# StephenTaf/Modern-Search-Engines-Project

Measured on AMD Instinct MI355X. Metric: queries/sec, two-stage retrieval top-100 (BM25 top-1000 + dense full scan + rerank/fuse), higher is better.
Workload: dtype f32 (exact f32 cosines of every returned document; candidates filtered by one pass of f16 products with a measured margin; batches <= 64 queries: f16x2-split products, |err| <= 8e-6) (dense cosine) / f64 (BM25, fuse)

## Files before the change

modern-search-engines-project_amd/csrc/msr_dense_ks.hip:

```cpp
#include <stdlib.h>

#include "msr_common.h"
#include "msr_internal.h"
#include "msr_frag.h"

namespace {

template <int QB, int MODE, int RING_DOCS = MSR_WIDE_RING, int NWAVES = 8> struct KsCfg {
    static constexpr int WAVES = NWAVES;
    static constexpr int THREADS = WAVES * 64;
    static constexpr int KS = MSR_DIM / 32;
    static constexpr int KT = KS / WAVES;
    static constexpr int PIECES = MODE == MODE_BF16 ? 1 : 2;
    static constexpr int NLU = MODE == MODE_BF16 ? KT : 2 * KT;
    static constexpr int ROW16 = MODE == MODE_BF16 ? MSR_DIM * 2 / 16 : MSR_DIM * 4 / 16;
    static constexpr int NQ = 16 * QB;
    static constexpr int RING = RING_DOCS;
    static constexpr int SWZ = (NQ < 64 ? NQ : 64) - 1;
    static constexpr int TILE = QB * 64 * 4;
    static constexpr int PER = QB / 2;
    static constexpr size_t p_bytes = (size_t)2 * WAVES * TILE * 4;
    static constexpr size_t r_bytes = (size_t)RING * NQ * 4;
    static constexpr size_t total = p_bytes + r_bytes;
    static_assert(QB == 2 || QB == 4 || QB == 8, "the reduction hands QB / 2 floats (one tile column piece) to a lane");
// ... 240 lines not shown
    }
}

int scan_debug_flags() {
#ifdef MSR_DIAG
    static const int v = [] { const char* e = getenv("MSR_SCAN_DEBUG"); return e ? atoi(e) : 0; }();
    return v;
#else
    return 0;
#endif
}

int ks_pipe_knob(int dflt) {
#ifdef MSR_DIAG
    static const char* v = getenv("MSR_KS_PIPE");
    return v ? atoi(v) : dflt;
#else
    return dflt;
#endif
}

template <int QB, int MODE, int NBUF, int PIPE = 1, int RING_DOCS = MSR_WIDE_RING, int NWAVES = 8>
hipError_t launch_ksplit(const DenseIndex& ix, const void* emb, const float* qn, int nq, float* docscore,
                         hipStream_t stream, int n_slices = 1, void* qimg_slices = nullptr) {
    using L = KsCfg<QB, MODE, RING_DOCS, NWAVES>;
    static_assert(L::total <= 160 * 1024, "LDS budget");
    hipError_t err = hipFuncSetAttribute((const void*)dense_ksplit_kernel<QB, MODE, NBUF, PIPE, RING_DOCS, NWAVES>,
                                         hipFuncAttributeMaxDynamicSharedMemorySize, (int)L::total);
    if (err != hipSuccess) return err;
    void* qimg = qimg_slices ? qimg_slices : ix.qimg;
    err = msr_build_qimage(MODE == MODE_PRE ? MODE_F16X2 : MODE, qn, QB * n_slices, qimg, stream);
    if (err != hipSuccess) return err;
    dense_ksplit_kernel<QB, MODE, NBUF, PIPE, RING_DOCS, NWAVES><<<dim3((unsigned)ix.n_spans, (unsigned)n_slices), L::THREADS,
                                                                 L::total, stream>>>(
        ix, emb, (const f32x4*)qimg, nq, docscore, scan_debug_flags());
    return hipGetLastError();
}

}

hipError_t msr_pack_row_meta(const int32_t* chunk_doc, const float* inv_norm, int64_t n, void* row_meta,
                             hipStream_t stream) {
    if (n <= 0) return hipSuccess;
    pack_row_meta_kernel<<<(unsigned)((n + 16 + 255) / 256), 256, 0, stream>>>(chunk_doc, inv_norm, n, (int2*)row_meta);
    return hipGetLastError();
}

hipError_t msr_presplit_rows(const float* src, int64_t n_rows, void* dst, hipStream_t stream) {
    if (n_rows <= 0) return hipSuccess;
    presplit_kernel<<<16384, 256, 0, stream>>>(src, n_rows, (f32x4*)dst);
    return hipGetLastError();
}

hipError_t msr_dense_scan_ksplit(const DenseIndex& ix, DensePlan plan, const float* qn, int nq, float* docscore,
// ... 4 lines not shown
        case dense_case(DENSE_KSPLIT_F16X2, 2): return launch_ksplit<2, MODE_F16X2, 3, 0>(ix, rows, qn, nq, docscore, stream);
        case dense_case(DENSE_KSPLIT_F16X2, 4):
#ifdef MSR_DIAG
            if (ks_pipe_knob(0) == 2) return launch_ksplit<4, MODE_F16X2, 3, 2>(ix, rows, qn, nq, docscore, stream);
            if (ks_pipe_knob(0) == 8) return launch_ksplit<4, MODE_F16X2, 3, 0>(ix, rows, qn, nq, docscore, stream);
#endif
            return launch_ksplit<4, MODE_F16X2, 2, 0, MSR_WIDE_RING, 12>(ix, rows, qn, nq, docscore, stream);
        case dense_case(DENSE_KSPLIT_PRESPLIT, 2): return launch_ksplit<2, MODE_PRE, 3, 0>(ix, rows, qn, nq, docscore, stream);
        case dense_case(DENSE_KSPLIT_PRESPLIT, 4): return launch_ksplit<4, MODE_PRE, 2, 0, MSR_WIDE_RING, 12>(ix, rows, qn, nq, docscore, stream);
        case dense_case(DENSE_KSPLIT_EXACT, 2): return launch_ksplit<2, MODE_F32, 3, 0>(ix, rows, qn, nq, docscore, stream);
        case dense_case(DENSE_KSPLIT_EXACT, 4): return launch_ksplit<4, MODE_F32, 2, 0, MSR_WIDE_RING, 12>(ix, rows, qn, nq, docscore, stream);
        case dense_case(DENSE_BF16_KSPLIT, 4):
#ifdef MSR_DIAG
            if (!ks_pipe_knob(1)) return launch_ksplit<4, MODE_BF16, 4, 0>(ix, rows, qn, nq, docscore, stream);
#endif
            return launch_ksplit<4, MODE_BF16, 4, 1>(ix, rows, qn, nq, docscore, stream);
        case dense_case(DENSE_BF16_KSPLIT, 8): return launch_ksplit<8, MODE_BF16, 3, 0, 64>(ix, rows, qn, nq, docscore, stream);
        default: break;
    }
    return hipErrorInvalidValue;
}

size_t msr_ksplit_slice_image_bytes() { return (size_t)4 * KsCfg<4, MODE_F16X2, MSR_WIDE_RING, 12>::KS * 2 * 64 * 16; }
hipError_t msr_dense_scan_slices(const DenseIndex& ix, const float* qn, int nq, float* docscore, void* qimg_slices,
                                 hipStream_t stream) {
    if (nq <= 0 || ix.n_docs <= 0) return hipSuccess;
    if (!dense_stream_bound(dense_binding(ix), true) || !ix.row_meta || !ix.gate || !qimg_slices) return hipErrorInvalidValue;
    static_assert(MSR_DENSE_FALLBACK_SLICE == 16 * 4, "a slice is what the QB = 4 instance below takes");
    return launch_ksplit<4, MODE_F16X2, 2, 0, MSR_WIDE_RING, 12>(ix, ix.emb, qn, nq, docscore, stream, dense_fallback_slices(nq),
                                                                 qimg_slices);
}
```

modern-search-engines-project_amd/csrc/msr_engine.hip:

```cpp
#include <hip/hip_runtime.h>
#include <stdarg.h>
#include <stdio.h>
#include <stdlib.h>
#include <string.h>

#include <algorithm>
#include <new>
#include <vector>

#include "../../include/msretr.h"
#include "msr_devmem.h"
#include "msr_internal.h"
#include "msr_match_args.h"

struct HipMem {
    static hipError_t alloc(void** p, size_t bytes) { return hipMalloc(p, bytes); }
    static void free(void* p) { (void)hipFree(p); }
};
using Group = DevGroup<HipMem>;

struct msr_engine {
    msr_config cfg;
    char err[512];
    Group mem_engine;
// ... 1315 lines not shown
                              (hipStream_t)stream));
    return MSR_OK;
}

extern "C" int msr_union_candidates(msr_engine* e, int32_t n_queries, const int32_t* lex_doc, const double* lex_score,
                                    const int32_t* lex_n, int32_t k_lex, const int32_t* dense_doc, const double* dense_bm25,
                                    const int32_t* dense_n, int32_t k_dense, int32_t* out_doc, double* out_score, int32_t* out_src,
                                    int32_t* out_n, int32_t max_cand, void* stream) {
    if (!e) return MSR_ERR_INVALID;
    if (n_queries < 0 || k_lex < 0 || k_lex > MSR_MAX_K || k_dense < 0 || k_dense > MSR_MAX_K || max_cand < 1 ||
        (int64_t)k_lex + k_dense > max_cand)
        return fail(e, MSR_ERR_INVALID, "msr_union_candidates: bad argument (k_lex=%d, k_dense=%d: each in [0, %d], their sum <= "
                    "max_cand=%d)", k_lex, k_dense, MSR_MAX_K, max_cand);
    if (!out_doc || !out_score || !out_src || !out_n || (k_lex > 0 && (!lex_doc || !lex_score || !lex_n)) ||
        (k_dense > 0 && (!dense_doc || !dense_bm25 || !dense_n)))
        return fail(e, MSR_ERR_INVALID, "msr_union_candidates: bad argument (NULL list)");
    if (n_queries == 0) return MSR_OK;
    HIP_TRY(e, hipSetDevice(e->cfg.device));
    HIP_TRY(e, msr_union_lists(n_queries, lex_doc, lex_score, lex_n, k_lex, dense_doc, dense_bm25, dense_n, k_dense, out_doc,
                               out_score, out_src, out_n, max_cand, (hipStream_t)stream));
    return MSR_OK;
}

static int dense_gated_fallback(msr_engine* e, int nq, int k, int32_t* out_doc, float* out_score, int32_t* out_chunk,
                                int32_t* out_n, hipStream_t st) {
    const int64_t N = e->dense.n_docs;
    DenseIndex ix = e->dense;
    ix.gate = e->gf_gate;
    HIP_TRY(e, msr_dense_scan_slices(ix, e->gf_qn, nq, (float*)e->score_rows, e->gf_fb_qimg, st));
    SelScratch sel = e->sel;
    sel.gate = e->gf_gate; sel.gate_per64 = 1;
    HIP_TRY(e, msr_select_topk(32, e->score_rows, N, e->dense.score_stride, nq, k, sel, out_doc, out_score, out_n, st));
    ix.gate = e->gf_gate; ix.gate_per64 = 1;
    if (out_chunk) HIP_TRY(e, msr_best_chunk(ix, e->gf_qn, nq, k, 0, out_doc, out_n, out_chunk, st));
    return MSR_OK;
}

static hipEvent_t* pass_events(msr_engine* e, int kind, hipEvent_t ev[4]) {
    if (!e->timing || e->ev_count[kind] >= msr_engine::EV_RING || e->ev_count[3] >= msr_engine::EV_RING) return nullptr;
    ev[0] = e->ev_start[3][e->ev_count[3]]; ev[1] = e->ev_stop[3][e->ev_count[3]];
    ev[2] = e->ev_start[kind][e->ev_count[kind]]; ev[3] = e->ev_stop[kind][e->ev_count[kind]];
    return ev;
}
static void pass_events_used(msr_engine* e, int kind, const hipEvent_t* ev) {
    if (ev) { e->ev_count[kind]++; e->ev_count[3]++; }
}

extern "C" int msr_dense_split_max(const msr_engine* e, int32_t k) {
    if (!e || !e->have_chunks || k < 1 || k > e->cfg.max_k ||
        !dense_stream_ok(dense_binding(e->dense), 0, e->gf_ok, e->gf.n_tiles, k))
        return 0;
    return e->gf.caps.call_cap;
}

extern "C" int msr_dense_topk_begin(msr_engine* e, const float* q, int32_t n_queries, int32_t k, int32_t k_part, float* out_part,
                                    void* stream) {
    if (!e) return MSR_ERR_INVALID;
    if (!e->have_chunks) return fail(e, MSR_ERR_NOT_BOUND, "msr_dense_topk_begin: chunks not bound");
    if (e->split_pending) return fail(e, MSR_ERR_INVALID, "msr_dense_topk_begin: the previous begin has not been ended");
    const int cap = msr_dense_split_max(e, k);
    if (!q || !out_part || k_part < 1 || k_part > k || n_queries <= 64 || n_queries > cap)
        return fail(e, MSR_ERR_INVALID, "msr_dense_topk_begin: needs 64 < n_queries <= msr_dense_split_max() = %d, 1 <= k_part <= k (got %d, %d, %d)",
                    cap, n_queries, k_part, k);
    hipStream_t st = (hipStream_t)stream;
    HIP_TRY(e, hipSetDevice(e->cfg.device));
    HIP_TRY(e, msr_prep_queries(q, n_queries, e->gf_qn, dense_fallback_pad(n_queries), st));
    HIP_TRY(e, hipMemsetAsync(e->gf_gate, 0, GF_GATE_BYTES, st));
    hipEvent_t ev_buf[4];
    hipEvent_t* ev = pass_events(e, 0, ev_buf);
    int width = 0;
    int segs = 0;
    HIP_TRY(e, msr_gemm_f32_pass(e->gf, e->dense, e->gf_qn, n_queries, k, k_part, out_part, ev, &width, &segs, st));
    e->last_dense_width = width;
    e->last_dense_segments = segs;
    pass_events_used(e, 0, ev);
    e->split_pending = n_queries;
    return MSR_OK;
}

extern "C" int msr_dense_topk_end(msr_engine* e, int32_t n_queries, int32_t k, const float* bound, int32_t* out_doc,
                                  float* out_score, int32_t* out_chunk, int32_t* out_n, void* stream) {
    if (!e) return MSR_ERR_INVALID;
    if (!e->have_chunks) return fail(e, MSR_ERR_NOT_BOUND, "msr_dense_topk_end: chunks not bound");
    if (!e->gf_ok || e->split_pending != n_queries || n_queries <= 0)
        return fail(e, MSR_ERR_INVALID, "msr_dense_topk_end: no matching msr_dense_topk_begin (pending %d, got %d)", e->split_pending, n_queries);
    if (!out_doc || !out_score || !out_n || k < 1 || k > e->cfg.max_k) return fail(e, MSR_ERR_INVALID, "msr_dense_topk_end: bad argument");
    e->split_pending = 0;
    hipStream_t st = (hipStream_t)stream;
    HIP_TRY(e, hipSetDevice(e->cfg.device));
    HIP_TRY(e, msr_gemm_f32_finish(e->gf, e->dense, e->gf_qn, n_queries, k, bound, out_doc, out_score, out_chunk, out_n, e->gf_gate, st));
// ... 34 lines not shown
                                      out_n + s0, out_chunk + (int64_t)s0 * k, st));
    }
    return MSR_OK;
}

extern "C" int msr_dense_topk(msr_engine* e, const float* q, int32_t n_queries, int32_t k, int32_t max_chunks_per_doc,
                              int32_t* out_doc, float* out_score, int32_t* out_chunk, int32_t* out_n, void* stream) {
    if (!e) return MSR_ERR_INVALID;
    const bool args_ok = dense_topk_args(e, n_queries, k, max_chunks_per_doc, q, out_doc, out_score, out_n);
    if (const int rc = dense_entry_ok(e, "msr_dense_topk", false, args_ok, k)) return rc;
    if (n_queries == 0) return MSR_OK;
    hipStream_t st = (hipStream_t)stream;
    HIP_TRY(e, hipSetDevice(e->cfg.device));
    const DenseBinding b = dense_binding(e->dense);
    const int slice = dense_slice(b, max_chunks_per_doc);
    const bool gemm = dense_stream_ok(b, max_chunks_per_doc, e->gf_ok, e->gf.n_tiles, k);
    e->last_dense_width = gemm && n_queries > slice ? 0 : slice;
    e->last_dense_segments = 0;
    int q0 = 0;
    while (q0 < n_queries) {
        const int left = n_queries - q0;
        if (gemm && left > slice) {
            const int nq = std::min(e->gf.caps.call_cap, left);
            HIP_TRY(e, msr_prep_queries(q + (int64_t)q0 * MSR_DIM, nq, e->gf_qn, dense_fallback_pad(nq), st));
            HIP_TRY(e, hipMemsetAsync(e->gf_gate, 0, GF_GATE_BYTES, st));
            hipEvent_t ev_buf[4];
            hipEvent_t* ev = pass_events(e, 0, ev_buf);
            int width = 0, segs = 0;
            HIP_TRY(e, msr_gemm_f32_topk(e->gf, e->dense, e->gf_qn, nq, k, out_doc + (int64_t)q0 * k,
                                         out_score + (int64_t)q0 * k, out_chunk ? out_chunk + (int64_t)q0 * k : nullptr,
                                         out_n + q0, e->gf_gate, ev, &width, &segs, st));
            e->last_dense_width = std::max(e->last_dense_width, width);
            e->last_dense_segments = segs;
            pass_events_used(e, 0, ev);
            {
                int rcf = dense_gated_fallback(e, nq, k, out_doc + (int64_t)q0 * k, out_score + (int64_t)q0 * k,
                                               out_chunk ? out_chunk + (int64_t)q0 * k : nullptr, out_n + q0, st);
                if (rcf) return rcf;
            }
            q0 += nq;
        } else {
            const int nq = std::min(slice, left);
            int rc = dense_sweeps(e, q, q0, nq, k, max_chunks_per_doc, nullptr, out_doc, out_score, out_chunk, out_n, st, nullptr);
            if (rc) return rc;
            q0 += nq;
        }
    }
    return MSR_OK;
// ... 511 lines not shown
```

modern-search-engines-project_amd/csrc/msr_gemm_f32.hip:

```cpp
#include <cmath>
#include <type_traits>

#include "msr_common.h"
#include "msr_internal.h"
#include "msr_frag.h"
#include "msr_gemm_dev.h"

namespace {

constexpr int GF_THREADS = 512;
constexpr int GF_KT = MSR_DIM / 32;
constexpr int GF_ROWB = MSR_DIM * 4;
constexpr int GF_PAIR_CAP = 4096;

typedef StreamArgs GemmF32Args;

__device__ __forceinline__ const char* uniform_ptr(const char* p) {
    const uint64_t u = (uint64_t)p;
    const uint32_t lo = __builtin_amdgcn_readfirstlane((uint32_t)u), hi = __builtin_amdgcn_readfirstlane((uint32_t)(u >> 32));
    return (const char*)(((uint64_t)hi << 32) | lo);
}

constexpr int GS_NB = 8;
constexpr int GS_STEP = 8192;
// ... 637 lines not shown
    if (i >= GF_KT * 256 * 4) return;
    const int g = blockIdx.y;
    const int cp = i & 3, ql = (i >> 2) & 255, kt = i >> 10;
    const int q = 256 * g + ql;
    const int c = cp ^ (((ql >> 3) & 1) << 1);
    f16x8 h;
    if (q < nq) {
        const float* src = qn + (size_t)q * MSR_DIM + (BF16 ? 64 * (kt >> 1) + 16 * c + 8 * (kt & 1) : 32 * kt + 8 * c);
        if (TOBF16) {
            bf16x8 b;
#pragma unroll
            for (int j = 0; j < 8; ++j) b[j] = (__bf16)src[j];
            h = __builtin_bit_cast(f16x8, b);
        } else {
            h = cvt_f16_rtn(*(const f32x4*)src, *(const f32x4*)(src + 4));
        }
    } else {
#pragma unroll
        for (int j = 0; j < 8; ++j) h[j] = (_Float16)0.f;
    }
    qimg[(size_t)g * (GF_KT * 256 * 4) + i] = h;
}

__global__ __launch_bounds__(256) void build_qimg1_kernel(const float* __restrict__ qn, int nq, f16x8* __restrict__ qimg) {
    const int i = blockIdx.x * 256 + threadIdx.x;
    if (i >= GF_KT * 128 * 4) return;
    const int g = blockIdx.y;
    const int cp = i & 3, ql = (i >> 2) & 127, kt = i >> 9;
    const int q = 128 * g + ql;
    const int c = cp ^ (((ql >> 3) & 1) << 1);
    f16x8 h;
    if (q < nq) {
        const float* src = qn + (size_t)q * MSR_DIM + 32 * kt + 8 * c;
        h = cvt_f16_rtn(*(const f32x4*)src, *(const f32x4*)(src + 4));
    } else {
#pragma unroll
        for (int j = 0; j < 8; ++j) h[j] = (_Float16)0.f;
    }
    qimg[(size_t)g * (GF_KT * 128 * 4) + i] = h;
}

__global__ __launch_bounds__(256) void pad_inv_kernel(const float* __restrict__ inv, int64_t n, int64_t n_pad, float* __restrict__ out) {
    const int64_t i = (int64_t)blockIdx.x * 256 + threadIdx.x;
    if (i < n_pad) out[i] = i < n ? inv[i] : 1.0f;
}

__global__ __launch_bounds__(256) void f16_row_error_kernel(const float* __restrict__ src, const float* __restrict__ inv_norm,
                                                             int64_t n_rows, uint32_t* __restrict__ err_max) {
    const int lane = threadIdx.x & 63;
    const int64_t wave = (int64_t)blockIdx.x * 4 + (threadIdx.x >> 6), n_waves = (int64_t)gridDim.x * 4;
    float worst = 0.f;
    for (int64_t r = wave; r < n_rows; r += n_waves) {
        const f32x4* p = (const f32x4*)(src + (size_t)r * MSR_DIM);
        float ss = 0.f;
#pragma unroll
        for (int h = 0; h < 3; ++h) {
            const f32x4 x = p[lane + 64 * h];
            ss += f16_err2(x.x) + f16_err2(x.y) + f16_err2(x.z) + f16_err2(x.w);
        }
        for (int o = 32; o > 0; o >>= 1) ss += __shfl_xor(ss, o);
        worst = fmaxf(worst, sqrtf(ss) * inv_norm[r]);
    }
    if (lane == 0) atomicMax(err_max, __float_as_uint(worst));
}

__global__ __launch_bounds__(256) void f16_margin_kernel(const float* __restrict__ qn, int nq, const uint32_t* __restrict__ err_max,
                                                          float* __restrict__ margin) {
    const int q = blockIdx.x * 4 + (threadIdx.x >> 6), lane = threadIdx.x & 63;
    if (q >= nq) return;
    float ss = 0.f;
    for (int j = lane; j < MSR_DIM; j += 64) ss += f16_err2(qn[(size_t)q * MSR_DIM + j]);
    for (int o = 32; o > 0; o >>= 1) ss += __shfl_xor(ss, o);
    if (lane == 0) {
        const float dq = sqrtf(ss) * 1.0001f, dE = __uint_as_float(*err_max) * 1.0001f;
        margin[q] = 2.0f * (dE * (1.0f + dq) + dq * 1.000001f) + 1.0e-4f;
    }
}

static_assert(GF_PAIR_CAP <= (1 << 13), "cand_first_len packs first and len into 13 bits each");
__global__ __launch_bounds__(1024) void gemm_f32_cand_kernel(int2* __restrict__ pairs, int32_t* __restrict__ pair_n,
                                                              const int32_t* __restrict__ chunk_doc, int64_t n_rows,
                                                              const int32_t* __restrict__ wv_count, int n_waves, int wv_cap,
                                                              const int32_t* __restrict__ flag, int32_t* __restrict__ cand_doc,
                                                              int32_t* __restrict__ cand_first_len,
                                                              int32_t* __restrict__ cand_n, int32_t* __restrict__ gate) {
    __shared__ uint64_t key[GF_PAIR_CAP];
    __shared__ int s_over, s_n;
    const int q = blockIdx.x, t = threadIdx.x;
    const int raw = pair_n[q];
    int over = raw > GF_PAIR_CAP || flag[q];
    for (int i = t; i < n_waves; i += 1024) over |= wv_count[i] > wv_cap;
    if (t == 0) { s_n = 0; s_over = 0; }
    __syncthreads();
    if (over) s_over = 1;
    __syncthreads();
    if (s_over) {
        if (t == 0) { cand_n[q] = 0; pair_n[q] = 0; atomicOr(gate + (q >> 6), 1); }
        return;
// ... 135 lines not shown
    return hipGetLastError();
}


hipError_t msr_f16_rows(const float* emb, int64_t n_rows, int64_t n_pad, void* out, hipStream_t stream) {
    if (n_pad <= 0) return hipSuccess;
    f16_rows_kernel<<<8192, 256, 0, stream>>>(emb, n_rows, n_pad, (f16x8*)out);
    return hipGetLastError();
}

hipError_t msr_pad_inv_norm(const float* inv, int64_t n, int64_t n_pad, float* out, hipStream_t stream) {
    if (n_pad <= 0) return hipSuccess;
    pad_inv_kernel<<<(unsigned)((n_pad + 255) / 256), 256, 0, stream>>>(inv, n, n_pad, out);
    return hipGetLastError();
}

hipError_t msr_f16_row_error(const float* emb, const float* inv_norm, int64_t n_rows, uint32_t* err_max, hipStream_t stream) {
    hipError_t err = hipMemsetAsync(err_max, 0, 4, stream);
    if (err != hipSuccess) return err;
    f16_row_error_kernel<<<8192, 256, 0, stream>>>(emb, inv_norm, n_rows, err_max);
    return hipGetLastError();
}

hipError_t msr_gemm_f32_pass(const GemmF32Index& g, const DenseIndex& ix, const float* qn, int nq, int k, int k_part,
                             float* out_part, hipEvent_t* ev, int* width_out, int* seg_out, hipStream_t stream) {
    StreamPlan p = stream_plan(g.caps, g.n_cus, nq, g.emb_tiled != nullptr, g.emb_f16 != nullptr);
#ifdef MSR_DIAG
    {
        StreamCaps c = g.caps;
        if (g_f32_dbg & 2048) c.max_nt = 1;
        if (g_f32_dbg & 4096) c.max_nt = std::min(c.max_nt, 2);
        p = stream_plan(c, g.n_cus, nq, g.emb_tiled != nullptr && !(g_f32_dbg & 8192),
                        g.emb_f16 != nullptr && !(g_f32_dbg & 1048576));
        if (g_f32_dbg & 16384) p.nt_loads = false;
        if (g_f32_dbg & 33554432) p.entry_tmax = false;
    }
#endif
    if (!p.valid || k < 1 || g.n_tiles < 2 * k) return hipErrorInvalidValue;
    const int W = p.W, G = p.G, NT = p.NT, grid = g.n_cus;
    const PassShape shape = pass_shape(g.n_tiles, k, grid, g.single_emit != 0);
    const int ss = shape.ss, n_s = shape.n_s;
    if (width_out) *width_out = W;
    if (seg_out) *seg_out = shape.n_seg;
    hipError_t err;
    switch (p.qimg) {
    case STREAM_QIMG_256_IMAGE16: build_qimg2_kernel<true, false><<<dim3((GF_KT * 256 * 4 + 255) / 256, G), 256, 0, stream>>>(qn, nq, (f16x8*)g.qimg); break;
    case STREAM_QIMG_256: build_qimg2_kernel<false><<<dim3((GF_KT * 256 * 4 + 255) / 256, G), 256, 0, stream>>>(qn, nq, (f16x8*)g.qimg); break;
    case STREAM_QIMG_128: build_qimg1_kernel<<<dim3((GF_KT * 128 * 4 + 255) / 256, G), 256, 0, stream>>>(qn, nq, (f16x8*)g.qimg); break;
    }
    f16_margin_kernel<<<(nq + 3) / 4, 256, 0, stream>>>(qn, nq, g.err_max, g.margin);
    const float* margin = g.margin;
    const size_t qimg_bytes = (size_t)GF_KT * W * 64;
    GemmF32Args a{};
    a.dbg = g_f32_dbg; a.nt = 1;
    a.E = (const char*)ix.emb; a.inv_pad = g.inv_pad; a.tile_row = g.tile_row;
    if (p.tiled) { a.E = (const char*)g.emb_tiled; a.tile_trow = g.tile_trow; }
    if (p.image16) a.E = (const char*)g.emb_f16;
    a.n_rows = ix.n_chunks; a.tmax_t = g.tmax_t;
    a.t_first = ss / 2; a.t_stride = ss; a.t_count = n_s;
    for (int gi = 0; gi < G; gi += NT) {
        a.nt = std::min(NT, G - gi);
        a.qimg = (const char*)g.qimg + gi * qimg_bytes;
        if (ev && gi == 0 && (err = hipEventRecord(ev[0], stream)) != hipSuccess) return err;
        if ((err = launch_f32(stream_kernel(p, a.nt), false, a, grid, stream)) != hipSuccess) return err;
        if (ev && gi == 0 && (err = hipEventRecord(ev[1], stream)) != hipSuccess) return err;
        if ((err = msr_gemm_tmax(g.tmax_t, n_s, p.tmax_parts, W * a.nt, g.tmax + (size_t)gi * W * g.tmax_stride, g.tmax_stride, stream)) != hipSuccess) return err;
    }
    if ((err = msr_gemm_kth(g.tmax, n_s, g.tmax_stride, nq, W * G, k, margin, g.thr, g.flag, stream)) != hipSuccess) return err;
    if (p.entry_tmax && (err = msr_gemm_tmax_clear(g.tmax, g.tmax_stride, W * G, stream)) != hipSuccess) return err;
    a.t_stride = 1;
    a.wvbuf = g.wvbuf; a.wv_cap = g.caps.wv_cap; a.wv_count = g.wv_count;
    for (int s = 0; s < shape.n_seg; ++s) {
        const int t0 = shape.bound[s], t1 = shape.bound[s + 1];
// ... 59 lines not shown
```

modern-search-engines-project_amd/csrc/msr_internal.h:

```cpp
#pragma once
#include <hip/hip_runtime.h>
#include <stdint.h>

#include "msr_dense_plan.h"
#include "msr_stream_plan.h"

#define MSR_DIM 768
#define MSR_SEL_BINS 4096
#define MSR_SEL_CAP 4096

struct SelState {
    uint64_t pref_hi, mask_hi;
    uint32_t pref_lo, mask_lo;
    int32_t k_rem;
    int32_t n_above;
    int32_t done;
    int32_t n_sel;
};

struct SelScratch {
    uint32_t* hist;
    SelState* state;
    uint64_t* cand_hi;
    uint32_t* cand_lo;
    int32_t* cand_n;
    const int32_t* gate;
    int gate_per64;
};

struct MsrSetView {
    const uint32_t* bits;
    int64_t stride;
    const int32_t* q_set;
    int32_t n_sets;
};
struct MsrSetRow {
    const uint32_t* bits;
    int32_t mode;
};
__device__ __forceinline__ MsrSetRow msr_set_row(int q, const MsrSetView& s) {
    const int32_t v = s.q_set[q];
    if (v == -1) return MsrSetRow{nullptr, 0};
    if (v < -1 || v >= s.n_sets) return MsrSetRow{nullptr, 2};
    return MsrSetRow{s.bits + (int64_t)v * s.stride, 1};
}
__device__ __forceinline__ bool msr_in_set(const MsrSetRow& r, int64_t d) {
    return r.mode == 0 || (r.mode == 1 && ((r.bits[d >> 5] >> (d & 31)) & 1u));
}

hipError_t msr_select_topk(int score_bits, const void* scores, int64_t n, int64_t stride, int nq, int k,
// ... 144 lines not shown
    int64_t score_stride;
    int32_t n_spans;
    int32_t layout;
    const int32_t* wspan_doc;
    int32_t n_wspans;
    void* qimg;
    const void* emb_bf16;
    const void* emb_presplit;
    const void* row_meta;
    int32_t wide_ok;
    int32_t wide_ok64;
    const int32_t* gate;
    int32_t variant;
    int32_t gate_per64;
};
inline DenseBinding dense_binding(const DenseIndex& ix) { return DenseBinding{ix.variant, ix.layout, ix.wide_ok, ix.wide_ok64}; }
hipError_t msr_dense_scan(const DenseIndex& ix, const float* qn, int nq, int max_chunks, float* docscore,
                          hipStream_t stream);
hipError_t msr_dense_scan_bf16(const DenseIndex& ix, const float* qn, int nq, int max_chunks, float* docscore,
                               hipStream_t stream);
hipError_t msr_dense_scan_ksplit(const DenseIndex& ix, DensePlan plan, const float* qn, int nq, float* docscore,
                                 hipStream_t stream);
size_t msr_ksplit_slice_image_bytes();
hipError_t msr_dense_scan_slices(const DenseIndex& ix, const float* qn, int nq, float* docscore, void* qimg_slices,
                                 hipStream_t stream);
hipError_t msr_build_qimage(int mode, const float* qn, int n_blocks, void* qimg, hipStream_t stream);
hipError_t msr_presplit_rows(const float* src, int64_t n_rows, void* dst, hipStream_t stream);
hipError_t msr_pack_row_meta(const int32_t* chunk_doc, const float* inv_norm, int64_t n, void* row_meta, hipStream_t stream);
hipError_t msr_fill_f32(float* dst, int64_t n, float value, hipStream_t stream);
hipError_t msr_inv_norm_range(const float* inv_norm, int64_t n, uint32_t* out2, hipStream_t stream);
hipError_t msr_prep_queries(const float* q, int nq, float* qn, int nq_pad, hipStream_t stream);
hipError_t msr_fill_chunk_doc(const int32_t* doc_off, int64_t n_docs, int32_t* chunk_doc, hipStream_t stream);
hipError_t msr_row_inv_norm(const float* emb, int64_t n_rows, float* inv_norm, hipStream_t stream);
hipError_t msr_interleave(const float* src, int64_t n_rows, float* dst, hipStream_t stream);
hipError_t msr_best_chunk(const DenseIndex& ix, const float* qn, int nq, int k, int max_chunks,
                          const int32_t* out_doc, const int32_t* out_n, int32_t* out_chunk, hipStream_t stream);

hipError_t msr_check_range(const int32_t* v, int64_t n, int64_t hi, int32_t* flag, hipStream_t stream);
hipError_t msr_gather_rows_run(const DenseIndex& ix, const int32_t* rows, int n, float* out, hipStream_t stream);
hipError_t msr_group_row_sets(const int32_t* group_off, int n_groups, const int32_t* g_set, int32_t* row_set, hipStream_t stream);
struct GroupedMergeArgs {
    const int32_t* l_doc; const float* l_score; const int32_t* l_chunk; const int32_t* l_n;
    int32_t kk;
    const int32_t* group_off;
    const int32_t* excl_off;
    const int32_t* excl_doc;
    int32_t k;
// ... 105 lines not shown
    void* qimg;
    float* tmax_t;
    float* tmax;
    int32_t tmax_stride;
    float* thr; float* thr2; int32_t* flag;
    void* wvbuf; int32_t* wv_count;
    void* pairs; int32_t* pair_n;
    uint32_t* err_max; float* margin;
    int32_t* cand_doc; float* cand_score; int32_t* cand_chunk; int32_t* cand_n;
    const void* emb_tiled;
    const int32_t* tile_trow;
    const void* emb_f16;
    int32_t single_emit;
};
hipError_t msr_f16_rows(const float* emb, int64_t n_rows, int64_t n_pad, void* out, hipStream_t stream);
hipError_t msr_tile_rows(const float* emb, const int32_t* tile_row, const int32_t* tile_trow, int n_tiles, void* emb_tiled,
                         hipStream_t stream);
hipError_t msr_f16_row_error(const float* emb, const float* inv_norm, int64_t n_rows, uint32_t* err_max, hipStream_t stream);
void msr_gemm_f32_set_dbg(int v);
hipError_t msr_pad_inv_norm(const float* inv, int64_t n, int64_t n_pad, float* out, hipStream_t stream);
hipError_t msr_gemm_f32_topk(const GemmF32Index& g, const DenseIndex& ix, const float* qn, int nq, int k,
                             int32_t* out_doc, float* out_score, int32_t* out_chunk,
                             int32_t* out_n, int32_t* gate, hipEvent_t* ev, int* width_out, int* seg_out, hipStream_t stream);
hipError_t msr_gemm_f32_pass(const GemmF32Index& g, const DenseIndex& ix, const float* qn, int nq, int k, int k_part,
                             float* out_part, hipEvent_t* ev, int* width_out, int* seg_out, hipStream_t stream);
hipError_t msr_gemm_f32_finish(const GemmF32Index& g, const DenseIndex& ix, const float* qn, int nq, int k, const float* bound,
                               int32_t* out_doc, float* out_score, int32_t* out_chunk, int32_t* out_n, int32_t* gate,
                               hipStream_t stream);

hipError_t msr_batch_rescore_rows(const DenseIndex& ix, const float* qn, int nq, int k, const int32_t* rows, int row_stride,
                                  int row_cap, int32_t* cand_doc, float* cand_score, int32_t* cand_chunk, int32_t* cand_n,
                                  int32_t* out_doc, float* out_score, int32_t* out_chunk, int32_t* out_n, hipStream_t stream);
hipError_t msr_batch_finish(const DenseIndex& ix, const float* qn, int nq, int k, int max_chunks, const float* margin,
                            const float* scores, const float* top_score, const int32_t* top_n, int32_t* cand_doc,
                            float* cand_score, int32_t* cand_chunk, int32_t* cand_n, int32_t* out_doc,
                            float* out_score, int32_t* out_chunk, int32_t* out_n, hipStream_t stream);
```

modern-search-engines-project_amd/csrc/msr_topk.hip:

```cpp
#include "msr_common.h"
#include "msr_internal.h"
#include "msr_sort.h"

#ifdef MSR_DIAG
__device__ unsigned long long msr_dbg_ts[16];
extern "C" int msr_debug_sel_final(unsigned long long* out16) {
    return (int)hipMemcpyFromSymbol(out16, HIP_SYMBOL(msr_dbg_ts), sizeof(unsigned long long) * 16);
}
#define DBG_TS(i) do { if (blockIdx.x == 0 && threadIdx.x == 0) msr_dbg_ts[i] = __builtin_readcyclecounter(); } while (0)
#else
#define DBG_TS(i) do { } while (0)
#endif

namespace {

constexpr int SEL_THREADS = 256;
constexpr int SCAN_THREADS = 1024;
constexpr int SEL_GRID = 2048;
constexpr int SEL_LIST_GRID = 4096;
constexpr int WIN_SHIFT = 44;

template <int SB> struct KeyCfg {
    static constexpr int NS = (SB + 11) / 12;
    static constexpr int ND = NS + 3;
// ... 341 lines not shown
        if (base + j < MSR_SEL_CAP) {
            cand_hi[(int64_t)q * MSR_SEL_CAP + base + j] = s_hi[j];
            cand_lo[(int64_t)q * MSR_SEL_CAP + base + j] = s_lo[j];
        }
    }
}

__device__ __forceinline__ bool key_less(uint64_t ah, uint32_t al, uint64_t bh, uint32_t bl) {
    return ah < bh || (ah == bh && al < bl);
}

using msr_sort::stage_sync;

template <typename T, typename... Set>
__global__ __launch_bounds__(SCAN_THREADS) void sel_final_kernel(const T* __restrict__ scores, int64_t n_dense,
                                                                  int64_t stride, RowView view,
                                                                  SelState* __restrict__ st,
                                                                  const uint64_t* __restrict__ cand_hi,
                                                                  const uint32_t* __restrict__ cand_lo,
                                                                  int32_t* __restrict__ cand_n, int k,
                                                                  int32_t* __restrict__ out_doc,
                                                                  T* __restrict__ out_score,
                                                                  int32_t* __restrict__ out_n,
                                                                  const int32_t* __restrict__ gate, int gate_per64, Set... set) {
    constexpr int SB = ScoreTraits<T>::SB;
    constexpr bool WITHIN = sizeof...(Set) > 0;
    if (gate && gate[gate_per64 ? (int)blockIdx.x >> 6 : 0] == 0) return;
    __shared__ uint64_t khi[MSR_SEL_CAP];
    __shared__ uint32_t klo[MSR_SEL_CAP];
    __shared__ uint32_t suf[SCAN_THREADS + 1];
    __shared__ SelState S_sh;
    __shared__ int s_cnt;
    const int q = blockIdx.x, t = threadIdx.x;
    const T* row = scores + (int64_t)q * stride;
    const int32_t* irow = view.idx ? view.idx + (int64_t)q * stride : nullptr;
    const MsrSetRow srow = sel_set_row(q, set...);
    int n_sg = 1, sg0 = 0;
    part_segments(view, 0, 1, sg0, n_sg);
    DBG_TS(0);
    if (t == 0) S_sh = st[q];
    __syncthreads();
    int cnt;
    DBG_TS(1);
    if (S_sh.done) {
        cnt = cand_n[q];
        if (cnt > MSR_SEL_CAP) cnt = MSR_SEL_CAP;
        const uint64_t* ch = cand_hi + (int64_t)q * MSR_SEL_CAP;
        const uint32_t* cl = cand_lo + (int64_t)q * MSR_SEL_CAP;
        int Pk = 64;
        while (Pk < k) Pk <<= 1;
        if (cnt <= Pk) {
            for (int i = t; i < cnt; i += SCAN_THREADS) { khi[i] = ch[i]; klo[i] = cl[i]; }
        } else {
            uint32_t* h = (uint32_t*)khi;
            int d = 0;
            for (; d < KeyCfg<SB>::ND; ++d) {
                int part, shift, width;
                digit_pos<SB>(d, part, shift, width);
                if (!(part == 0 ? (S_sh.mask_hi >> shift) & 1 : (S_sh.mask_lo >> shift) & 1)) break;
            }
            int cur = cnt;
            for (; cur > Pk && d < KeyCfg<SB>::ND; ++d) {
                for (int b = t; b < MSR_SEL_BINS; b += SCAN_THREADS) h[b] = 0;
// ... 96 lines not shown
    }
    if (t == 0) {
        out_n[q] = n_sel;
        cand_n[q] = 0;
    }
    DBG_TS(5);
#ifdef MSR_DIAG
    if (blockIdx.x == 0 && t == 0) { msr_dbg_ts[6] = (unsigned long long)cnt; msr_dbg_ts[7] = (unsigned long long)P; }
#endif
}

template <typename T, typename... Set>
hipError_t select_impl(const T* scores, int64_t n, int64_t stride, RowView view, int nq, int k, const SelScratch& sc,
                       int32_t* out_doc, T* out_score, int32_t* out_n, hipStream_t stream, Set... set) {
    constexpr int SB = ScoreTraits<T>::SB;
    if (nq <= 0) return hipSuccess;
    int64_t parts = view.counts ? view.n_seg : (n + 8191) / 8192;
    const int grid_cap = view.counts ? SEL_LIST_GRID : SEL_GRID;
    const int64_t max_parts = grid_cap / nq > 0 ? grid_cap / nq : 1;
    if (parts > max_parts) parts = max_parts;
    if (parts < 1) parts = 1;
    dim3 grid((unsigned)parts, (unsigned)nq);
    const bool window = SB == 64 && view.win_base != nullptr;
    for (int d = window ? -1 : 0; d < (window ? 0 : 2); ++d) {
        sel_hist_kernel<T, Set...><<<grid, SEL_THREADS, 0, stream>>>(scores, n, stride, view, d, sc.state, sc.hist, sc.gate,
                                                                     sc.gate_per64, set...);
        sel_scan_kernel<SB><<<nq, SCAN_THREADS, 0, stream>>>(sc.state, sc.hist, d, k, sc.gate, sc.gate_per64, view.win_base);
    }
    sel_compact_kernel<T, Set...><<<grid, SEL_THREADS, 0, stream>>>(scores, n, stride, view, sc.state, sc.cand_hi, sc.cand_lo,
                                                                     sc.cand_n, sc.gate, sc.gate_per64, set...);
    sel_final_kernel<T, Set...><<<nq, SCAN_THREADS, 0, stream>>>(scores, n, stride, view, sc.state, sc.cand_hi, sc.cand_lo,
                                                                  sc.cand_n, k, out_doc, out_score, out_n, sc.gate, sc.gate_per64,
                                                                  set...);
    return hipGetLastError();
}

template <typename T>
__global__ __launch_bounds__(SCAN_THREADS) void merge_kernel(const int32_t* __restrict__ in_doc,
                                                              const T* __restrict__ in_score,
                                                              const int32_t* __restrict__ in_n,
                                                              const int32_t* __restrict__ in_pay, int n_parts,
                                                              int64_t pstride, int nq, int k, int32_t* __restrict__ out_doc,
                                                              T* __restrict__ out_score,
                                                              int32_t* __restrict__ out_n,
                                                              int32_t* __restrict__ out_pay, int only_left_over) {
    extern __shared__ __attribute__((aligned(16))) char smem[];
    const int q = blockIdx.x;
    if (only_left_over && out_n[q] != -1) return;
    int lg = 6;
    while ((1 << lg) < k) ++lg;
    const int Pk = 1 << lg;
    int NP = 1;
    while (NP < n_parts) NP <<= 1;
    const int P = NP * Pk;
    uint64_t* khi = (uint64_t*)smem;
    uint32_t* klo = (uint32_t*)(smem + (size_t)P * 8);
// ... 284 lines not shown
```

Before: 70370.

## Fuse query normalization, image build, margin and gate reset into one prep kernel

Replaces the separate query normalization, hipMemset of the gate, per-pass f16 query-image build, margin kernel and fallback slice-image build with a single stream_prep_kernel launched once per call. The dense fallback no longer rebuilds its slice image and runs only the final selection kernel from scratch, skipping the histogram/scan/compact passes. This is meant to cut kernel launch overhead and redundant passes in small-batch queries. The final-only selection relies on the final kernel handling the full candidate set alone, which could be slower or wrong if the fallback yields many candidates.

```diff
diff --git a/modern-search-engines-project_amd/csrc/msr_dense_ks.hip b/modern-search-engines-project_amd/csrc/msr_dense_ks.hip
--- a/modern-search-engines-project_amd/csrc/msr_dense_ks.hip
+++ b/modern-search-engines-project_amd/csrc/msr_dense_ks.hip
@@ -286,14 +286,14 @@
 
 template <int QB, int MODE, int NBUF, int PIPE = 1, int RING_DOCS = MSR_WIDE_RING, int NWAVES = 8>
 hipError_t launch_ksplit(const DenseIndex& ix, const void* emb, const float* qn, int nq, float* docscore,
-                         hipStream_t stream, int n_slices = 1, void* qimg_slices = nullptr) {
+                         hipStream_t stream, int n_slices = 1, void* qimg_slices = nullptr, bool image_built = false) {
     using L = KsCfg<QB, MODE, RING_DOCS, NWAVES>;
     static_assert(L::total <= 160 * 1024, "LDS budget");
     hipError_t err = hipFuncSetAttribute((const void*)dense_ksplit_kernel<QB, MODE, NBUF, PIPE, RING_DOCS, NWAVES>,
                                          hipFuncAttributeMaxDynamicSharedMemorySize, (int)L::total);
     if (err != hipSuccess) return err;
     void* qimg = qimg_slices ? qimg_slices : ix.qimg;
-    err = msr_build_qimage(MODE == MODE_PRE ? MODE_F16X2 : MODE, qn, QB * n_slices, qimg, stream);
+    if (!image_built) err = msr_build_qimage(MODE == MODE_PRE ? MODE_F16X2 : MODE, qn, QB * n_slices, qimg, stream);
     if (err != hipSuccess) return err;
     dense_ksplit_kernel<QB, MODE, NBUF, PIPE, RING_DOCS, NWAVES><<<dim3((unsigned)ix.n_spans, (unsigned)n_slices), L::THREADS,
                                                                  L::total, stream>>>(
@@ -344,11 +344,11 @@
 }
 
 size_t msr_ksplit_slice_image_bytes() { return (size_t)4 * KsCfg<4, MODE_F16X2, MSR_WIDE_RING, 12>::KS * 2 * 64 * 16; }
-hipError_t msr_dense_scan_slices(const DenseIndex& ix, const float* qn, int nq, float* docscore, void* qimg_slices,
+hipError_t msr_dense_scan_slices(const DenseIndex& ix, const float* qn, int nq, float* docscore, const void* qimg_slices,
                                  hipStream_t stream) {
     if (nq <= 0 || ix.n_docs <= 0) return hipSuccess;
     if (!dense_stream_bound(dense_binding(ix), true) || !ix.row_meta || !ix.gate || !qimg_slices) return hipErrorInvalidValue;
     static_assert(MSR_DENSE_FALLBACK_SLICE == 16 * 4, "a slice is what the QB = 4 instance below takes");
     return launch_ksplit<4, MODE_F16X2, 2, 0, MSR_WIDE_RING, 12>(ix, ix.emb, qn, nq, docscore, stream, dense_fallback_slices(nq),
-                                                                 qimg_slices);
-}
+                                                                 const_cast<void*>(qimg_slices), true);
+}
diff --git a/modern-search-engines-project_amd/csrc/msr_engine.hip b/modern-search-engines-project_amd/csrc/msr_engine.hip
--- a/modern-search-engines-project_amd/csrc/msr_engine.hip
+++ b/modern-search-engines-project_amd/csrc/msr_engine.hip
@@ -1361,6 +1361,11 @@
     return MSR_OK;
 }
 
+static hipError_t dense_stream_prep(msr_engine* e, const float* q, int nq, hipStream_t st) {
+    return msr_gemm_f32_prep(e->gf, q, nq, e->gf_qn, dense_fallback_pad(nq), e->gf_fb_qimg, e->gf_gate,
+                             (int)(GF_GATE_BYTES / sizeof(int32_t)), st);
+}
+
 static int dense_gated_fallback(msr_engine* e, int nq, int k, int32_t* out_doc, float* out_score, int32_t* out_chunk,
                                 int32_t* out_n, hipStream_t st) {
     const int64_t N = e->dense.n_docs;
@@ -1369,6 +1374,7 @@
     HIP_TRY(e, msr_dense_scan_slices(ix, e->gf_qn, nq, (float*)e->score_rows, e->gf_fb_qimg, st));
     SelScratch sel = e->sel;
     sel.gate = e->gf_gate; sel.gate_per64 = 1;
+    sel.final_only = 1;
     HIP_TRY(e, msr_select_topk(32, e->score_rows, N, e->dense.score_stride, nq, k, sel, out_doc, out_score, out_n, st));
     ix.gate = e->gf_gate; ix.gate_per64 = 1;
     if (out_chunk) HIP_TRY(e, msr_best_chunk(ix, e->gf_qn, nq, k, 0, out_doc, out_n, out_chunk, st));
@@ -1403,8 +1409,7 @@
                     cap, n_queries, k_part, k);
     hipStream_t st = (hipStream_t)stream;
     HIP_TRY(e, hipSetDevice(e->cfg.device));
-    HIP_TRY(e, msr_prep_queries(q, n_queries, e->gf_qn, dense_fallback_pad(n_queries), st));
-    HIP_TRY(e, hipMemsetAsync(e->gf_gate, 0, GF_GATE_BYTES, st));
+    HIP_TRY(e, dense_stream_prep(e, q, n_queries, st));
     hipEvent_t ev_buf[4];
     hipEvent_t* ev = pass_events(e, 0, ev_buf);
     int width = 0;
@@ -1485,8 +1490,7 @@
         const int left = n_queries - q0;
         if (gemm && left > slice) {
             const int nq = std::min(e->gf.caps.call_cap, left);
-            HIP_TRY(e, msr_prep_queries(q + (int64_t)q0 * MSR_DIM, nq, e->gf_qn, dense_fallback_pad(nq), st));
-            HIP_TRY(e, hipMemsetAsync(e->gf_gate, 0, GF_GATE_BYTES, st));
+            HIP_TRY(e, dense_stream_prep(e, q + (int64_t)q0 * MSR_DIM, nq, st));
             hipEvent_t ev_buf[4];
             hipEvent_t* ev = pass_events(e, 0, ev_buf);
             int width = 0, segs = 0;
diff --git a/modern-search-engines-project_amd/csrc/msr_gemm_f32.hip b/modern-search-engines-project_amd/csrc/msr_gemm_f32.hip
--- a/modern-search-engines-project_amd/csrc/msr_gemm_f32.hip
+++ b/modern-search-engines-project_amd/csrc/msr_gemm_f32.hip
@@ -683,24 +683,6 @@
     qimg[(size_t)g * (GF_KT * 256 * 4) + i] = h;
 }
 
-__global__ __launch_bounds__(256) void build_qimg1_kernel(const float* __restrict__ qn, int nq, f16x8* __restrict__ qimg) {
-    const int i = blockIdx.x * 256 + threadIdx.x;
-    if (i >= GF_KT * 128 * 4) return;
-    const int g = blockIdx.y;
-    const int cp = i & 3, ql = (i >> 2) & 127, kt = i >> 9;
-    const int q = 128 * g + ql;
-    const int c = cp ^ (((ql >> 3) & 1) << 1);
-    f16x8 h;
-    if (q < nq) {
-        const float* src = qn + (size_t)q * MSR_DIM + 32 * kt + 8 * c;
-        h = cvt_f16_rtn(*(const f32x4*)src, *(const f32x4*)(src + 4));
-    } else {
-#pragma unroll
-        for (int j = 0; j < 8; ++j) h[j] = (_Float16)0.f;
-    }
-    qimg[(size_t)g * (GF_KT * 128 * 4) + i] = h;
-}
-
 __global__ __launch_bounds__(256) void pad_inv_kernel(const float* __restrict__ inv, int64_t n, int64_t n_pad, float* __restrict__ out) {
     const int64_t i = (int64_t)blockIdx.x * 256 + threadIdx.x;
     if (i < n_pad) out[i] = i < n ? inv[i] : 1.0f;
@@ -725,16 +707,69 @@
     if (lane == 0) atomicMax(err_max, __float_as_uint(worst));
 }
 
-__global__ __launch_bounds__(256) void f16_margin_kernel(const float* __restrict__ qn, int nq, const uint32_t* __restrict__ err_max,
-                                                          float* __restrict__ margin) {
-    const int q = blockIdx.x * 4 + (threadIdx.x >> 6), lane = threadIdx.x & 63;
-    if (q >= nq) return;
+template <bool BF16K>
+__global__ __launch_bounds__(256) void stream_prep_kernel(const float* __restrict__ q, int nq, int nq_pad, int n_img, int W,
+                                                           float* __restrict__ qn, const uint32_t* __restrict__ err_max,
+                                                           float* __restrict__ margin, f16x8* __restrict__ qimg,
+                                                           f32x4* __restrict__ fb_qimg, int32_t* __restrict__ gate,
+                                                           int gate_words) {
+    __shared__ __attribute__((aligned(16))) float s_q[4][MSR_DIM];
+    const int w = threadIdx.x >> 6, lane = threadIdx.x & 63;
+    const int row = blockIdx.x * 4 + w;
+    if (blockIdx.x == 0 && (int)threadIdx.x < gate_words) gate[threadIdx.x] = 0;
+    float v[12];
     float ss = 0.f;
-    for (int j = lane; j < MSR_DIM; j += 64) ss += f16_err2(qn[(size_t)q * MSR_DIM + j]);
-    for (int o = 32; o > 0; o >>= 1) ss += __shfl_xor(ss, o);
-    if (lane == 0) {
-        const float dq = sqrtf(ss) * 1.0001f, dE = __uint_as_float(*err_max) * 1.0001f;
-        margin[q] = 2.0f * (dE * (1.0f + dq) + dq * 1.000001f) + 1.0e-4f;
+    for (int j = 0; j < 12; ++j) {
+        v[j] = row < nq ? q[(size_t)row * MSR_DIM + lane + 64 * j] : 0.f;
+        ss += v[j] * v[j];
+    }
+    for (int off = 32; off > 0; off >>= 1) ss += __shfl_xor(ss, off);
+    float nrm = sqrtf(ss);
+    if (nrm == 0.f) nrm = 1.f;
+    for (int j = 0; j < 12; ++j) {
+        v[j] = v[j] / nrm;
+        if (row < nq_pad) qn[(size_t)row * MSR_DIM + lane + 64 * j] = v[j];
+        s_q[w][lane + 64 * j] = v[j];
+    }
+    if (row < nq) {
+        float es = 0.f;
+        for (int j = 0; j < 12; ++j) es += f16_err2(v[j]);
+        for (int o = 32; o > 0; o >>= 1) es += __shfl_xor(es, o);
+        if (lane == 0) {
+            const float dq = sqrtf(es) * 1.0001f, dE = __uint_as_float(*err_max) * 1.0001f;
+            margin[row] = 2.0f * (dE * (1.0f + dq) + dq * 1.000001f) + 1.0e-4f;
+        }
+    }
+    __syncthreads();
+    const float* src = s_q[w];
+    if (row < n_img) {
+        const int g = row / W, ql = row - g * W;
+        for (int p = lane; p < GF_KT * 4; p += 64) {
+            const int kt = p >> 2, cp = p & 3;
+            const int c = cp ^ (((ql >> 3) & 1) << 1);
+            const float* s8 = src + (BF16K ? 64 * (kt >> 1) + 16 * c + 8 * (kt & 1) : 32 * kt + 8 * c);
+            f16x8 h;
+            if (row < nq) {
+                h = cvt_f16_rtn(*(const f32x4*)s8, *(const f32x4*)(s8 + 4));
+            } else {
+#pragma unroll
+                for (int j = 0; j < 8; ++j) h[j] = (_Float16)0.f;
+            }
+            qimg[(size_t)g * (GF_KT * W * 4) + ((size_t)kt * W + ql) * 4 + cp] = h;
+        }
+    }
+    if (fb_qimg && row < nq_pad) {
+        constexpr int KS = MSR_DIM / 32;
+        const int qb = row >> 4, i = row & 15;
+        for (int p = lane; p < KS * 4; p += 64) {
+            const int t = p >> 2, g4 = p & 3, l = i + 16 * g4;
+            const f32x4 a = *(const f32x4*)(src + 16 * (2 * t) + 4 * g4);
+            const f32x4 b = *(const f32x4*)(src + 16 * (2 * t + 1) + 4 * g4);
+            f16x8 hi, lo;
+            split_f16(a, b, hi, lo);
+            fb_qimg[((size_t)qb * KS + t) * 128 + l] = __builtin_bit_cast(f32x4, hi);
+            fb_qimg[((size_t)qb * KS + t) * 128 + 64 + l] = __builtin_bit_cast(f32x4, lo);
+        }
     }
 }
 
@@ -916,8 +951,7 @@
     return hipGetLastError();
 }
 
-hipError_t msr_gemm_f32_pass(const GemmF32Index& g, const DenseIndex& ix, const float* qn, int nq, int k, int k_part,
-                             float* out_part, hipEvent_t* ev, int* width_out, int* seg_out, hipStream_t stream) {
+static StreamPlan call_plan(const GemmF32Index& g, int nq) {
     StreamPlan p = stream_plan(g.caps, g.n_cus, nq, g.emb_tiled != nullptr, g.emb_f16 != nullptr);
 #ifdef MSR_DIAG
     {
@@ -930,6 +964,27 @@
         if (g_f32_dbg & 33554432) p.entry_tmax = false;
     }
 #endif
+    return p;
+}
+
+hipError_t msr_gemm_f32_prep(const GemmF32Index& g, const float* q, int nq, float* qn, int nq_pad, void* fb_qimg, int32_t* gate,
+                             int gate_words, hipStream_t stream) {
+    const StreamPlan p = call_plan(g, nq);
+    if (!p.valid || nq_pad < nq || gate_words < 0 || gate_words > 256) return hipErrorInvalidValue;
+    const int n_img = p.W * p.G;
+    const unsigned blocks = (unsigned)((std::max(n_img, nq_pad) + 3) / 4);
+    if (p.qimg == STREAM_QIMG_256_IMAGE16)
+        stream_prep_kernel<true><<<blocks, 256, 0, stream>>>(q, nq, nq_pad, n_img, p.W, qn, g.err_max, g.margin, (f16x8*)g.qimg,
+                                                             (f32x4*)fb_qimg, gate, gate_words);
+    else
+        stream_prep_kernel<false><<<blocks, 256, 0, stream>>>(q, nq, nq_pad, n_img, p.W, qn, g.err_max, g.margin, (f16x8*)g.qimg,
+                                                              (f32x4*)fb_qimg, gate, gate_words);
+    return hipGetLastError();
+}
+
+hipError_t msr_gemm_f32_pass(const GemmF32Index& g, const DenseIndex& ix, const float* qn, int nq, int k, int k_part,
+                             float* out_part, hipEvent_t* ev, int* width_out, int* seg_out, hipStream_t stream) {
+    const StreamPlan p = call_plan(g, nq);
     if (!p.valid || k < 1 || g.n_tiles < 2 * k) return hipErrorInvalidValue;
     const int W = p.W, G = p.G, NT = p.NT, grid = g.n_cus;
     const PassShape shape = pass_shape(g.n_tiles, k, grid, g.single_emit != 0);
@@ -937,12 +992,6 @@
     if (width_out) *width_out = W;
     if (seg_out) *seg_out = shape.n_seg;
     hipError_t err;
-    switch (p.qimg) {
-    case STREAM_QIMG_256_IMAGE16: build_qimg2_kernel<true, false><<<dim3((GF_KT * 256 * 4 + 255) / 256, G), 256, 0, stream>>>(qn, nq, (f16x8*)g.qimg); break;
-    case STREAM_QIMG_256: build_qimg2_kernel<false><<<dim3((GF_KT * 256 * 4 + 255) / 256, G), 256, 0, stream>>>(qn, nq, (f16x8*)g.qimg); break;
-    case STREAM_QIMG_128: build_qimg1_kernel<<<dim3((GF_KT * 128 * 4 + 255) / 256, G), 256, 0, stream>>>(qn, nq, (f16x8*)g.qimg); break;
-    }
-    f16_margin_kernel<<<(nq + 3) / 4, 256, 0, stream>>>(qn, nq, g.err_max, g.margin);
     const float* margin = g.margin;
     const size_t qimg_bytes = (size_t)GF_KT * W * 64;
     GemmF32Args a{};
diff --git a/modern-search-engines-project_amd/csrc/msr_internal.h b/modern-search-engines-project_amd/csrc/msr_internal.h
--- a/modern-search-engines-project_amd/csrc/msr_internal.h
+++ b/modern-search-engines-project_amd/csrc/msr_internal.h
@@ -26,6 +26,7 @@
     int32_t* cand_n;
     const int32_t* gate;
     int gate_per64;
+    int final_only;
 };
 
 struct MsrSetView {
@@ -216,7 +217,7 @@
 hipError_t msr_dense_scan_ksplit(const DenseIndex& ix, DensePlan plan, const float* qn, int nq, float* docscore,
                                  hipStream_t stream);
 size_t msr_ksplit_slice_image_bytes();
-hipError_t msr_dense_scan_slices(const DenseIndex& ix, const float* qn, int nq, float* docscore, void* qimg_slices,
+hipError_t msr_dense_scan_slices(const DenseIndex& ix, const float* qn, int nq, float* docscore, const void* qimg_slices,
                                  hipStream_t stream);
 hipError_t msr_build_qimage(int mode, const float* qn, int n_blocks, void* qimg, hipStream_t stream);
 hipError_t msr_presplit_rows(const float* src, int64_t n_rows, void* dst, hipStream_t stream);
@@ -368,6 +369,8 @@
 hipError_t msr_gemm_f32_topk(const GemmF32Index& g, const DenseIndex& ix, const float* qn, int nq, int k,
                              int32_t* out_doc, float* out_score, int32_t* out_chunk,
                              int32_t* out_n, int32_t* gate, hipEvent_t* ev, int* width_out, int* seg_out, hipStream_t stream);
+hipError_t msr_gemm_f32_prep(const GemmF32Index& g, const float* q, int nq, float* qn, int nq_pad, void* fb_qimg, int32_t* gate,
+                             int gate_words, hipStream_t stream);
 hipError_t msr_gemm_f32_pass(const GemmF32Index& g, const DenseIndex& ix, const float* qn, int nq, int k, int k_part,
                              float* out_part, hipEvent_t* ev, int* width_out, int* seg_out, hipStream_t stream);
 hipError_t msr_gemm_f32_finish(const GemmF32Index& g, const DenseIndex& ix, const float* qn, int nq, int k, const float* bound,
diff --git a/modern-search-engines-project_amd/csrc/msr_topk.hip b/modern-search-engines-project_amd/csrc/msr_topk.hip
--- a/modern-search-engines-project_amd/csrc/msr_topk.hip
+++ b/modern-search-engines-project_amd/csrc/msr_topk.hip
@@ -387,7 +387,8 @@
                                                                   int32_t* __restrict__ out_doc,
                                                                   T* __restrict__ out_score,
                                                                   int32_t* __restrict__ out_n,
-                                                                  const int32_t* __restrict__ gate, int gate_per64, Set... set) {
+                                                                  const int32_t* __restrict__ gate, int gate_per64,
+                                                                  int from_scratch, Set... set) {
     constexpr int SB = ScoreTraits<T>::SB;
     constexpr bool WITHIN = sizeof...(Set) > 0;
     if (gate && gate[gate_per64 ? (int)blockIdx.x >> 6 : 0] == 0) return;
@@ -403,7 +404,16 @@
     int n_sg = 1, sg0 = 0;
     part_segments(view, 0, 1, sg0, n_sg);
     DBG_TS(0);
-    if (t == 0) S_sh = st[q];
+    if (t == 0) {
+        if (from_scratch) {
+            SelState S;
+            S.pref_hi = S.mask_hi = 0; S.pref_lo = S.mask_lo = 0;
+            S.k_rem = k; S.n_above = 0; S.done = 0; S.n_sel = 0;
+            S_sh = S;
+        } else {
+            S_sh = st[q];
+        }
+    }
     __syncthreads();
     int cnt;
     DBG_TS(1);
@@ -546,6 +556,12 @@
     if (parts < 1) parts = 1;
     dim3 grid((unsigned)parts, (unsigned)nq);
     const bool window = SB == 64 && view.win_base != nullptr;
+    if (sc.final_only) {
+        sel_final_kernel<T, Set...><<<nq, SCAN_THREADS, 0, stream>>>(scores, n, stride, view, sc.state, sc.cand_hi, sc.cand_lo,
+                                                                      sc.cand_n, k, out_doc, out_score, out_n, sc.gate,
+                                                                      sc.gate_per64, 1, set...);
+        return hipGetLastError();
+    }
     for (int d = window ? -1 : 0; d < (window ? 0 : 2); ++d) {
         sel_hist_kernel<T, Set...><<<grid, SEL_THREADS, 0, stream>>>(scores, n, stride, view, d, sc.state, sc.hist, sc.gate,
                                                                      sc.gate_per64, set...);
@@ -555,7 +571,7 @@
                                                                      sc.cand_n, sc.gate, sc.gate_per64, set...);
     sel_final_kernel<T, Set...><<<nq, SCAN_THREADS, 0, stream>>>(scores, n, stride, view, sc.state, sc.cand_hi, sc.cand_lo,
                                                                   sc.cand_n, k, out_doc, out_score, out_n, sc.gate, sc.gate_per64,
-                                                                  set...);
+                                                                  0, set...);
     return hipGetLastError();
 }
 
```

Result: no change. 70860 (median of 6 runs) (+0.7%).
